# terraytherapeutics/COATI

Measured on AMD Instinct MI355X. Metric: molecules/sec (contrastive+AR train step), grande_closed, higher is better.
Workload: dtype bf16; 1 GPU; grande_closed d=256 L=16 nh=16 + E3GNN h=256x5, V=10322, batch 1024/GPU, seq_len 80, 16-atom point clouds, InfoNCE + AR loss, bf16 MFMA operands / fp32 accumulate + fp32 master weights, random-init weights; global_batch=1024, seq_len=80, parallelism=dp1

## Files before the change

### coati_amd/_lib.py

```python
import ctypes
import os

from . import _abi
from . import build as _build

try:
    with open(_build.HEADER) as _f:
        _ABI = _abi.parse(_f.read())
except OSError as e:
    raise RuntimeError(f"coati_amd: cannot read {_build.HEADER}, which the binding of libcoati_hip.so is derived from: {e}") from e
try:
    with open(_build.BEAM_HEADER) as _f:
        _BEAM_ABI = _abi.parse(_f.read(), guard="COATI_BEAM_H", name="coati_beam.h", base=_ABI)
except OSError as e:
    raise RuntimeError(f"coati_amd: cannot read {_build.BEAM_HEADER}, which the beam-search binding is derived from: {e}") from e
try:
    with open(_build.SEARCH_HEADER) as _f:
        _SEARCH_ABI = _abi.parse(_f.read(), guard="COATI_SEARCH_H", name="coati_search.h", base=_ABI)
except OSError as e:
    raise RuntimeError(f"coati_amd: cannot read {_build.SEARCH_HEADER}, which the library-search binding is derived from: {e}") from e
try:
    with open(_build.GRAMMAR_HEADER) as _f:
        _GRAMMAR_ABI = _abi.parse(_f.read(), guard="COATI_GRAMMAR_H", name="coati_grammar.h", base=_ABI)
except OSError as e:
# ... 61 lines not shown
try:
    with open(_build.PQ_HEADER) as _f:
        _PQ_ABI = _abi.parse(_f.read(), guard="COATI_PQ_H", name="coati_pq.h", base=_ABI)
except OSError as e:
    raise RuntimeError(f"coati_amd: cannot read {_build.PQ_HEADER}, which the binding of the product-quantised search is derived from: {e}") from e
try:
    with open(_build.IVFPQ_HEADER) as _f:
        _IVFPQ_ABI = _abi.parse(_f.read(), guard="COATI_IVFPQ_H", name="coati_ivfpq.h", base=_ABI)
except OSError as e:
    raise RuntimeError(f"coati_amd: cannot read {_build.IVFPQ_HEADER}, which the binding of the IVF-PQ search is derived from: {e}") from e
try:
    with open(_build.SEARCH4_HEADER) as _f:
        _SEARCH4_ABI = _abi.parse(_f.read(), guard="COATI_SEARCH4_H", name="coati_search4.h", base=_ABI)
except OSError as e:
    raise RuntimeError(f"coati_amd: cannot read {_build.SEARCH4_HEADER}, which the binding of the four-bit search is derived from: {e}") from e

PROTOTYPES = _ABI.prototypes
CoatiConfig = _ABI.CoatiConfig
ABI_VERSION = _ABI.version
BEAM_PROTOTYPES = _BEAM_ABI.prototypes
SEARCH_PROTOTYPES = _SEARCH_ABI.prototypes
GRAMMAR_PROTOTYPES = _GRAMMAR_ABI.prototypes
SCREEN_PROTOTYPES = _SCREEN_ABI.prototypes
GUIDE_PROTOTYPES = _GUIDE_ABI.prototypes
LN_XHAT_PROTOTYPES = _LN_XHAT_ABI.prototypes
GP_PROTOTYPES = _GP_ABI.prototypes
ACQ_PROTOTYPES = _ACQ_ABI.prototypes
CLUSTER_PROTOTYPES = _CLUSTER_ABI.prototypes
IVF_PROTOTYPES = _IVF_ABI.prototypes
RADIUS_PROTOTYPES = _RADIUS_ABI.prototypes
GNN_OPS_PROTOTYPES = _GNN_OPS_ABI.prototypes
SEARCH8_PROTOTYPES = _SEARCH8_ABI.prototypes
IVF8_PROTOTYPES = _IVF8_ABI.prototypes
IVF_RADIUS_PROTOTYPES = _IVF_RADIUS_ABI.prototypes
PQ_PROTOTYPES = _PQ_ABI.prototypes
IVFPQ_PROTOTYPES = _IVFPQ_ABI.prototypes
SEARCH4_PROTOTYPES = _SEARCH4_ABI.prototypes

_lib = None


def has_experimental():
    return hasattr(lib(), "coati_attn_block_fwd")


def lib():
    global _lib
    if _lib is not None:
        return _lib
    path = _build.LIB
    try:
        _build.build(force=os.environ.get("COATI_AMD_REBUILD") == "1", verbose=False)
    except Exception:
        if not os.path.exists(path):
            raise
    if not os.path.exists(path):
        raise RuntimeError(f"coati_amd: {path} is missing and could not be built; there is no CPU fallback")
    import torch
    l = ctypes.CDLL(path)
    for name, (restype, argtypes) in list(PROTOTYPES.items()) + list(BEAM_PROTOTYPES.items()) + list(SEARCH_PROTOTYPES.items()) + list(GRAMMAR_PROTOTYPES.items()) + list(SCREEN_PROTOTYPES.items()) + list(GUIDE_PROTOTYPES.items()) + list(LN_XHAT_PROTOTYPES.items()) + list(GP_PROTOTYPES.items()) + list(ACQ_PROTOTYPES.items()) + list(CLUSTER_PROTOTYPES.items()) + list(IVF_PROTOTYPES.items()) + list(RADIUS_PROTOTYPES.items()) + list(GNN_OPS_PROTOTYPES.items()) + list(SEARCH8_PROTOTYPES.items()) + list(IVF8_PROTOTYPES.items()) + list(IVF_RADIUS_PROTOTYPES.items()) + list(PQ_PROTOTYPES.items()) + list(IVFPQ_PROTOTYPES.items()) + list(SEARCH4_PROTOTYPES.items()):
        if hasattr(l, name):
            getattr(l, name).restype = restype
            getattr(l, name).argtypes = argtypes
    if l.coati_abi_version() != ABI_VERSION:
        raise RuntimeError(f"coati_amd: {path} has ABI version {l.coati_abi_version()}, this package expects {ABI_VERSION}; "
                           "rebuild with `python -m coati_amd.build --force`")
    missing = [n for n in exported_symbols() + sorted(BEAM_PROTOTYPES) + sorted(SEARCH_PROTOTYPES) + sorted(GRAMMAR_PROTOTYPES) + sorted(SCREEN_PROTOTYPES) + sorted(GUIDE_PROTOTYPES) + sorted(LN_XHAT_PROTOTYPES) + sorted(GP_PROTOTYPES) + sorted(ACQ_PROTOTYPES) + sorted(CLUSTER_PROTOTYPES) + sorted(IVF_PROTOTYPES) + sorted(RADIUS_PROTOTYPES) + sorted(GNN_OPS_PROTOTYPES) + sorted(SEARCH8_PROTOTYPES) + sorted(IVF8_PROTOTYPES) + sorted(IVF_RADIUS_PROTOTYPES) + sorted(PQ_PROTOTYPES) + sorted(IVFPQ_PROTOTYPES) + sorted(SEARCH4_PROTOTYPES) if not hasattr(l, n)]
    if missing:
        raise RuntimeError(f"coati_amd: {path} lacks symbols {missing[:6]}; rebuild with `python -m coati_amd.build --force`")
    _lib = l
    return l


def exported_symbols():
    return sorted(n for n in PROTOTYPES if _build.EXPERIMENTAL or n not in _ABI.experimental)


def check(rc, what=""):
    if rc != 0:
        msg = lib().coati_last_error().decode("utf-8", "replace")
        raise RuntimeError(f"libcoati_hip: {what} failed (code {rc}): {msg}")

# ... 6 lines not shown
```

### coati_amd/build.py

```python
import os
import subprocess
import sys
from concurrent.futures import ThreadPoolExecutor

HERE = os.path.dirname(os.path.abspath(__file__))
CSRC = os.path.join(HERE, "csrc")
LIBDIR = os.path.join(HERE, "lib")
LIB = os.path.join(LIBDIR, "libcoati_hip_x.so" if os.environ.get("COATI_AMD_EXPERIMENTAL") == "1" else "libcoati_hip.so")
OBJDIR = os.path.join(HERE, "build")
HEADER = os.path.join(os.path.dirname(HERE), "include", "coati_hip.h")
BEAM_HEADER = os.path.join(os.path.dirname(HERE), "include", "coati_beam.h")
SEARCH_HEADER = os.path.join(os.path.dirname(HERE), "include", "coati_search.h")
GRAMMAR_HEADER = os.path.join(os.path.dirname(HERE), "include", "coati_grammar.h")
SCREEN_HEADER = os.path.join(os.path.dirname(HERE), "include", "coati_screen.h")
GUIDE_HEADER = os.path.join(os.path.dirname(HERE), "include", "coati_guide.h")
LN_XHAT_HEADER = os.path.join(os.path.dirname(HERE), "include", "coati_ln_xhat.h")
GP_HEADER = os.path.join(os.path.dirname(HERE), "include", "coati_gp.h")
ACQ_HEADER = os.path.join(os.path.dirname(HERE), "include", "coati_acq.h")
CLUSTER_HEADER = os.path.join(os.path.dirname(HERE), "include", "coati_cluster.h")
IVF_HEADER = os.path.join(os.path.dirname(HERE), "include", "coati_ivf.h")
RADIUS_HEADER = os.path.join(os.path.dirname(HERE), "include", "coati_radius.h")
GNN_OPS_HEADER = os.path.join(os.path.dirname(HERE), "include", "coati_gnn_ops.h")
SEARCH8_HEADER = os.path.join(os.path.dirname(HERE), "include", "coati_search8.h")
IVF8_HEADER = os.path.join(os.path.dirname(HERE), "include", "coati_ivf8.h")
IVF_RADIUS_HEADER = os.path.join(os.path.dirname(HERE), "include", "coati_ivf_radius.h")
PQ_HEADER = os.path.join(os.path.dirname(HERE), "include", "coati_pq.h")
IVFPQ_HEADER = os.path.join(os.path.dirname(HERE), "include", "coati_ivfpq.h")
SEARCH4_HEADER = os.path.join(os.path.dirname(HERE), "include", "coati_search4.h")
HIP_UNITS = ["gemm.hip", "gemm_rb.hip", "gemm_rb16.hip", "gemm_ring.hip", "gemm_mx8.hip", "norm.hip", "attention.hip", "attention16.hip", "embed.hip", "gnn.hip", "loss.hip", "optim.hip", "batch.hip", "decode.hip", "beam.hip", "search.hip", "grammar.hip", "screen.hip", "guide.hip", "gp.hip", "gp_grad.hip", "cluster.hip", "ivf.hip", "radius.hip", "search8.hip", "ivf8.hip", "ivf_radius.hip", "pq.hip", "ivfpq.hip", "search4.hip"]
CPP_UNITS = ["engine.cpp", "capi.cpp", "tokenizer.cpp", "comm.cpp"]
FLAGS = ["--offload-arch=gfx950", "-O3", "-std=c++17", "-fPIC", "-Wno-unused-value", "-mllvm", "-amdgpu-mfma-vgpr-form=1"] + os.environ.get("COATI_AMD_CXXFLAGS", "").split()


EXPERIMENTAL = os.environ.get("COATI_AMD_EXPERIMENTAL") == "1"
EXPERIMENTAL_UNITS = ["experimental/attn_block.hip", "experimental/mlp64.hip", "experimental/gemm_t32.hip"]
if EXPERIMENTAL:
    HIP_UNITS = HIP_UNITS + EXPERIMENTAL_UNITS
    FLAGS = FLAGS + ["-DCOATI_EXPERIMENTAL"]
UNIT_DROP_FLAGS = {"experimental/mlp64.hip": ("-mllvm", "-amdgpu-mfma-vgpr-form=1")}


def _hipcc():
    for c in (os.environ.get("HIPCC"), "/opt/rocm/bin/hipcc", "hipcc"):
        if c and (os.path.isabs(c) and os.path.exists(c) or not os.path.isabs(c)):
            return c
    return "hipcc"


def _sources():
    deps = [os.path.join(CSRC, f) for f in os.listdir(CSRC) if not os.path.isdir(os.path.join(CSRC, f))]
    if EXPERIMENTAL:
        deps += [os.path.join(CSRC, "experimental", f) for f in os.listdir(os.path.join(CSRC, "experimental"))]
    deps += [HEADER, BEAM_HEADER, SEARCH_HEADER, GRAMMAR_HEADER, SCREEN_HEADER, GUIDE_HEADER, LN_XHAT_HEADER, GP_HEADER, ACQ_HEADER, CLUSTER_HEADER, IVF_HEADER, RADIUS_HEADER, GNN_OPS_HEADER, SEARCH8_HEADER, IVF8_HEADER, IVF_RADIUS_HEADER, PQ_HEADER, IVFPQ_HEADER, SEARCH4_HEADER]
    return deps


def _stamp_path():
    return LIB + ".flags"


def needs_build():
    if not os.path.exists(LIB):
        return True
    try:
        with open(_stamp_path()) as f:
            if f.read() != " ".join(FLAGS):
                return True
    except OSError:
# ... 51 lines not shown
```

### coati_amd/csrc/capi.cpp

```cpp
#include <string.h>

#include "../../include/coati_hip.h"
#include "../../include/coati_beam.h"
#include "../../include/coati_search.h"
#include "../../include/coati_grammar.h"
#include "../../include/coati_screen.h"
#include "../../include/coati_guide.h"
#include "../../include/coati_ln_xhat.h"
#include "../../include/coati_gp.h"
#include "../../include/coati_acq.h"
#include "../../include/coati_cluster.h"
#include "../../include/coati_ivf.h"
#include "../../include/coati_radius.h"
#include "../../include/coati_search8.h"
#include "../../include/coati_ivf8.h"
#include "../../include/coati_ivf_radius.h"
#include "../../include/coati_pq.h"
#include "../../include/coati_ivfpq.h"
#include "../../include/coati_search4.h"
#include "../../include/coati_gnn_ops.h"
#include <vector>
#include "kernels.h"

#define S_(x) ((hipStream_t)(x))
#define LL(x) (reinterpret_cast<const long long*>(x))

extern "C" {

int coati_gemm_nt(const void* A, int a_f32, int64_t lda, const uint16_t* B, int64_t ldb, int M, int N, int K,
                  void* C, int64_t ldc, int n_store, const float* bias, const void* aux_in, void* aux_out,
                  int64_t ld_aux, int epi, void* stream) {
  COATI_CHECK_ARG((epi >= EPI_BF16 && epi <= EPI_ACC_F32) || epi == EPI_GELU_GRAD || epi == EPI_MUL_AUX, "coati_gemm_nt: epilogue %d is not a plain epilogue", epi);
  GemmArgs a;
  memset(&a, 0, sizeof(a));
  a.A = A; a.lda = lda; a.B = B; a.ldb = ldb; a.M = M; a.N = N; a.K = K; a.C = C; a.ldc = ldc; a.n_store = n_store;
// ... 445 lines not shown
}
int coati_gnn_edge_reduce(const uint16_t* s2, const int32_t* seg, const float* e_w, uint16_t* mi, int64_t ldmi, int BA, int H, void* stream) {
  return launch_gnn_edge_reduce_c(s2, seg, e_w, mi, ldmi, BA, H, S_(stream));
}

int coati_gnn_edge_fwd_fused(const uint16_t* P, int64_t ldp, const int32_t* seg, const int32_t* e_bk, const float* e_d2, const float* e_w,
                             const float* w1c, int64_t w1c_stride, const float* b1, const uint16_t* W3, int64_t ldw, const float* b3,
                             uint16_t* e1, uint16_t* s2, uint16_t* mi, int64_t ldmi, int BA, int H, void* stream) {
  return launch_gnn_edge_fwd_fused(P, ldp, seg, e_bk, e_d2, e_w, w1c, w1c_stride, b1, W3, ldw, b3, e1, s2, mi, ldmi, BA, H, S_(stream));
}
int coati_gnn_edge_reduce_bwd(const uint16_t* dmi, int64_t lddmi, const uint16_t* s2, const int32_t* seg, const float* e_w, uint16_t* ds2,
                              int BA, int H, void* stream) {
  COATI_CHECK_SHAPE(BA > 0 && H > 0, "gnn_edge_reduce_bwd: empty problem");
  return launch_gnn_edge_reduce_bwd_c(dmi, lddmi, s2, seg, e_w, ds2, BA, H, S_(stream));
}
int coati_gnn_edge_pre_bwd(const uint16_t* dpre, const int32_t* seg, const int32_t* e_rev, const float* e_d2, uint16_t* dP, int64_t lddp,
                           float* dw1c, int64_t dw1c_stride, float* db1, int BA, int H, void* stream) {
  COATI_CHECK_SHAPE(BA > 0 && H > 0, "gnn_edge_pre_bwd: empty problem");
  return launch_gnn_edge_pre_bwd_c(dpre, seg, e_rev, e_d2, dP, lddp, dw1c, dw1c_stride, db1, BA, H, S_(stream));
}
int coati_gnn_node_res_silu(const float* u32, const int64_t* atoms, const int32_t* lut_ix, const int32_t* lut_iy, const float* W3c,
                            int64_t ldw, uint16_t* upre, uint16_t* t16, int BA, int H, void* stream) {
  COATI_CHECK_SHAPE(BA > 0 && H > 0, "gnn_node_res_silu: empty problem");
  return launch_gnn_node_res_silu(u32, LL(atoms), lut_ix, lut_iy, W3c, ldw, upre, t16, BA, H, S_(stream));
}
int coati_gnn_onehot_wgrad(const int64_t* atoms, const int32_t* lut_ix, const int32_t* lut_iy, const uint16_t* du, float* dW, int64_t ldw,
                           int BA, int H, void* stream) {
  COATI_CHECK_SHAPE(BA > 0 && H > 0, "gnn_onehot_wgrad: empty problem");
  return launch_gnn_onehot_wgrad(LL(atoms), lut_ix, lut_iy, du, dW, ldw, BA, H, S_(stream));
}
// ... 100 lines not shown
```

### coati_amd/csrc/engine.cpp

```cpp
#include <stdarg.h>
#include <stdio.h>
#include <stdlib.h>
#include <string.h>

#include <algorithm>
#include <string>
#include <vector>

#include "../../include/coati_hip.h"
#include "../../include/coati_beam.h"
#include "../../include/coati_ln_xhat.h"
#include "kernels.h"

#define HIPCHK(x) do { hipError_t _h = (x); if (_h != hipSuccess) { coati_set_error("%s: %s", #x, hipGetErrorString(_h)); return COATI_EHIP; } } while (0)

static thread_local char g_err[512] = "";
void coati_set_error(const char* fmt, ...) {
  va_list ap;
  va_start(ap, fmt);
  vsnprintf(g_err, sizeof(g_err), fmt, ap);
  va_end(ap);
}
extern "C" const char* coati_last_error(void) { return g_err; }
extern "C" int coati_abi_version(void) { return COATI_ABI_VERSION; }
// ... 1218 lines not shown
    bf16_t* const du = grp ? e->gl_du[l] : e->g_du;
    bf16_t* const dP = grp ? e->gl_dP[l] : e->g_dP;
    {
      ProfScope ps(e, SITE_GNN_ELEMWISE, 0, s, (double)BA * (H * 4 + H * 4 + 4 + H * 4 + H * 2));
      COATI_TRY(launch_layernorm_bwd(DH, 1, H, e->g_h32[l + 1], H, 1, nullptr, e->g_rstd[l + 1], nullptr, nullptr, DO, DO16, nullptr, nullptr, e->ln_partial, BA, H, s));
    }
    COATI_TRY(gemm(e, SITE_GNN_NODE_GEMM, DO16, 0, H, e->S + w.n3T, H, BA, H, H, du, H, nullptr, EPI_DSILU, e->g_upre[l], nullptr, H, s));
    if (!grp) COATI_TRY(wgrad(e, SITE_GNN_WGRAD, DO16, 0, H, e->g_t[l], H, BA, H, H, e->G + w.n3w, H, e->G + w.n3b, 0, s));
    COATI_TRY(gemm(e, SITE_GNN_NODE_GEMM, du, 0, H, e->S + w.n0T, H, BA, H, H, DO, H, nullptr, EPI_ACC_F32, nullptr, nullptr, 0, s));
    COATI_TRY(gemm(e, SITE_GNN_NODE_GEMM, du, 0, H, e->S + w.n0T + (int64_t)H * H, H, BA, H, H, e->g_dmi, H, nullptr, EPI_BF16, nullptr, nullptr, 0, s));
    if (!grp) COATI_TRY(wgrad(e, SITE_GNN_WGRAD, du, 0, H, e->g_hcat[l], 2 * H, BA, H, 2 * H, e->G + w.n0w, 2 * H + (c.residual ? 28 : 0), e->G + w.n0b, 0, s));
    if (c.residual) {
      ProfScope ps(e, SITE_GNN_ELEMWISE, 0, s, (double)BA * (H * 2 + 8));
      COATI_TRY(launch_gnn_onehot_wgrad(e->atoms, e->lut_ix, e->lut_iy, du, e->G + w.n0w + 2 * H, 2 * H + 28, BA, H, s));
    }
    {
      ProfScope ps(e, SITE_GNN_ELEMWISE, 0, s, (double)BA * (H * 2 + 4), (double)H * 4 + 4, 6.0 * H);
      COATI_TRY(launch_gnn_edge_reduce_bwd_c(e->g_dmi, H, e->g_s2[l], e->g_seg, e->g_ew, e->g_ds2, BA, H, s));
    }
    {
      GemmArgs a;
      memset(&a, 0, sizeof(a));
      a.A = e->g_ds2; a.lda = H; a.B = e->S + w.e3T; a.ldb = H; a.M = Me; a.N = H; a.K = H; a.C = e->g_dpre1; a.ldc = H;
      a.P = e->g_P[l]; a.ldp = 2 * H; a.d2 = e->g_ed2; a.w1c = e->P + w.e0w + 2 * H; a.w1c_stride = 2 * H + 1;
      a.b1 = e->P + w.e0b; a.natom = A; a.H = H;
      a.m_dev = e->g_ne; a.e_bj = e->g_ebj; a.e_bk = e->g_ebk;
      ProfScope ps(e, SITE_GNN_EDGE_GEMM, 0, s, (double)H * H * 2, (double)H * 8 + 12, 2.0 * H * H + 8.0 * H);
      COATI_TRY(launch_gemm_nt(a, 0, EPI_EDGE_DPRE, s));
    }
    {
      WgradArgs a;
      a.A = e->g_ds2; a.lda = H; a.B = e->g_e1[l]; a.ldb = H; a.M = Me; a.N = H; a.K = H; a.dW = e->G + w.e3w; a.ldw = H; a.dbias = e->G + w.e3b;
      a.n_out = 0; a.m_dev = e->g_ne;
      ProfScope ps(e, SITE_GNN_WGRAD, 0, s, (double)H * H * 8, (double)H * 4, 2.0 * H * H);
      COATI_TRY(launch_wgrad(a, 0, s));
    }
    {
      ProfScope ps(e, SITE_GNN_ELEMWISE, 0, s, (double)BA * (H * 4 + 4), (double)H * 4 + 8, 4.0 * H);
      COATI_TRY(launch_gnn_edge_pre_bwd_c(e->g_dpre1, e->g_seg, e->g_erev, e->g_ed2, dP, 2 * H, e->G + w.e0w + 2 * H, 2 * H + 1, e->G + w.e0b, BA, H, s));
    }
    COATI_TRY(gemm(e, SITE_GNN_NODE_GEMM, dP, 0, 2 * H, e->S + w.w1abT, 2 * H, BA, H, 2 * H, DO, H, nullptr, EPI_ACC_F32, nullptr, nullptr, 0, s));
    if (!grp) {
      COATI_TRY(wgrad(e, SITE_GNN_WGRAD, dP, 0, 2 * H, e->g_hcat[l], 2 * H, BA, H, H, e->G + w.e0w, 2 * H + 1, nullptr, 0, s));
// ... 1192 lines not shown
```

### coati_amd/csrc/gemm_rb16.hip

```cpp
#include <algorithm>
#include <cstdlib>
#include "gemm_epi.h"

#define R16_K 256
#define R16_BN 64
#define R16_TILE_HALFS (R16_BN * R16_K)
#define R16_BIAS_MAX 4096
#define R16_MAXW 16
#ifndef R16_TURNS
#define R16_TURNS 4
#endif
#ifndef R16_PRIO
#define R16_PRIO 0
#endif
#ifndef R16_ABLATE
#define R16_ABLATE 0
#endif
typedef float f32x4_t __attribute__((ext_vector_type(4)));
typedef unsigned r16_v4u __attribute__((ext_vector_type(4)));
#if R16_ABLATE & 16
__device__ unsigned char r16_sink[512 * 4096];
#endif

template <typename F>
// ... 335 lines not shown
    sm += __shfl_xor(sm, 16, 64);
    sm += __shfl_xor(sm, 32, 64);
    if (rowok && kq == 0) p.lse_out[row_l] = mx + __logf(sm);
    if (p.tl_out != nullptr) {
      float tl = ce_tl + __shfl_xor(ce_tl, 16, 64);
      tl += __shfl_xor(tl, 32, 64);
      if (rowok && kq == 0) p.tl_out[row_l] = tl;
    }
  }
#if R16_ABLATE & 16
#undef p
#endif
}

#define R16_RES_TILES 4
template <int EPI>
__global__ __launch_bounds__(64 * R16_MAXW, 1) void gemm_rb16_resident_kernel(GemmArgs p) {
  extern __shared__ __attribute__((aligned(16))) unsigned char smem[];
  constexpr int MAP = 0;
  bf16_t* const Bs = reinterpret_cast<bf16_t*>(smem);
  float* const BiasS = reinterpret_cast<float*>(smem + R16_RES_TILES * R16_TILE_HALFS * 2);
  float* const ColS = BiasS + R16_RES_TILES * R16_BN;
  const int tid = threadIdx.x, lane = tid & 63, wave = __builtin_amdgcn_readfirstlane(tid >> 6), W = blockDim.x >> 6;
  const int fr = lane & 15, kq = lane >> 4;
  const int ntiles = (p.N + R16_BN - 1) / R16_BN;
  const int M = __builtin_amdgcn_readfirstlane(p.m_dev != nullptr ? *p.m_dev : p.M);
  const bool has_bias = p.bias != nullptr;
  if (M <= 0) return;
  for (int c = tid; c < ntiles * R16_BN; c += blockDim.x) {
    BiasS[c] = (has_bias && c < p.N) ? p.bias[c] : 0.f;
// ... 10 lines not shown
    const int gc = r < p.N ? r : p.N - 1;
    const bf16_t* src = p.B + (long long)gc * p.ldb + ((q ^ r16_swz<MAP>(r & 63)) * 8);
    __builtin_amdgcn_global_load_lds((gbl_void*)src, (lds_void*)(Bs + k * 512), 16, 0, 0);
  }
  __builtin_amdgcn_s_waitcnt(0x0f70);
  __syncthreads();

  int wofs[4], wsw[4];
#pragma unroll
  for (int a = 0; a < 4; ++a) {
    const int n = r16_wrow<MAP>(a, fr);
    wofs[a] = n * R16_K;
    wsw[a] = r16_swz<MAP>(n);
  }
  const int colA = 8 * kq, colB = 32 + 8 * kq;
  GemmArgs q = p;
  q.bias = nullptr;
  q.M = M;

  const int slabs = (M + 15) / 16, per_wg = (slabs + (int)gridDim.x - 1) / (int)gridDim.x;
  const int s_begin = blockIdx.x * per_wg, s_end = s_begin + per_wg < slabs ? s_begin + per_wg : slabs;
  for (int sl = s_begin + wave; sl < s_end; sl += W) {
    const int m0 = sl * 16, row_l = m0 + fr, rc = row_l < M ? row_l : M - 1;
    const bool rowok = row_l < M;
    bf16x8 af[8];
    {
      const bf16_t* ap = reinterpret_cast<const bf16_t*>(p.A) + (long long)rc * p.lda + kq * 8;
#pragma unroll
      for (int ks = 0; ks < 8; ++ks) af[ks] = *reinterpret_cast<const bf16x8*>(ap + ks * 32);
    }
    for (int jt = 0; jt < ntiles; ++jt) {
      const bf16_t* cur = Bs + jt * R16_TILE_HALFS;
      f32x4_t acc[4];
      acc[0] = *reinterpret_cast<const f32x4_t*>(BiasS + jt * R16_BN + colA);
      acc[1] = *reinterpret_cast<const f32x4_t*>(BiasS + jt * R16_BN + colA + 4);
      acc[2] = *reinterpret_cast<const f32x4_t*>(BiasS + jt * R16_BN + colB);
      acc[3] = *reinterpret_cast<const f32x4_t*>(BiasS + jt * R16_BN + colB + 4);
      {
        constexpr int WFD = (EPI == EPI_EDGE_DPRE) ? 1 : 2;
// ... 6 lines not shown
#pragma unroll
            for (int a = 0; a < 4; ++a) wf[(ks + 1) % WFD][a] = *reinterpret_cast<const bf16x8*>(cur + wofs[a] + (((4 * (ks + 1) + kq) ^ wsw[a]) * 8));
          }
#pragma unroll
          for (int a = 0; a < 4; ++a) acc[a] = __builtin_amdgcn_mfma_f32_16x16x32_bf16(wf[ks % WFD][a], af[ks], acc[a], 0, 0, 0);
          if (WFD == 1 && ks + 1 < 8) {
#pragma unroll
            for (int a = 0; a < 4; ++a) wf[0][a] = *reinterpret_cast<const bf16x8*>(cur + wofs[a] + (((4 * (ks + 1) + kq) ^ wsw[a]) * 8));
          }
          __builtin_amdgcn_sched_barrier(0);
        }
      }
      float v0[8] = {acc[0][0], acc[0][1], acc[0][2], acc[0][3], acc[1][0], acc[1][1], acc[1][2], acc[1][3]};
      float v1[8] = {acc[2][0], acc[2][1], acc[2][2], acc[2][3], acc[3][0], acc[3][1], acc[3][2], acc[3][3]};
      const int c0 = jt * R16_BN + colA, c1 = jt * R16_BN + colB;
      const void* st0 = nullptr;
      const void* st1 = nullptr;
      if constexpr (EPI == EPI_EDGE_DPRE) { st0 = ColS + jt * 128 + colA; st1 = ColS + jt * 128 + colB; }
      epilogue8<EPI>(q, row_l, c0, v0, rowok, jt, ntiles, st0);
      __builtin_amdgcn_sched_barrier(0);
      epilogue8<EPI>(q, row_l, c1, v1, rowok, jt, ntiles, st1);
    }
  }
}

bool gemm_rb16_resident_supported(const GemmArgs& a, int a_f32, int epi) {
  if (a_f32 || a.K != R16_K || a.m_dev == nullptr) return false;
  if (epi != EPI_BF16 && epi != EPI_EDGE_DPRE) return false;
  if (a.N % 16 != 0 || a.N > R16_RES_TILES * R16_BN || a.q8_out != nullptr || a.ln_x != nullptr) return false;
  return a.M >= 16 * 256;
}

template <int EPI>
static int launch_rb16_resident_t(const GemmArgs& a, hipStream_t s) {
  static bool attr_set = false;
  auto kern = gemm_rb16_resident_kernel<EPI>;
  constexpr size_t lds = (size_t)R16_RES_TILES * R16_TILE_HALFS * 2 + (size_t)R16_RES_TILES * R16_BN * 4 + (size_t)R16_RES_TILES * 128 * 4;
  if (!attr_set) {
    if (hipFuncSetAttribute(reinterpret_cast<const void*>(kern), hipFuncAttributeMaxDynamicSharedMemorySize, (int)lds) != hipSuccess) {
      coati_set_error("gemm_rb16(resident): hipFuncSetAttribute failed");
      return COATI_EHIP;
    }
    attr_set = true;
  }
  hipLaunchKernelGGL(kern, dim3(256), dim3(64 * R16_MAXW), lds, s, a);
  COATI_LAUNCH_CHECK("gemm_rb16_resident");
  return COATI_OK;
}

int launch_gemm_rb16_resident(const GemmArgs& a, int epi, hipStream_t s) {
  if (epi == EPI_EDGE_DPRE) return launch_rb16_resident_t<EPI_EDGE_DPRE>(a, s);
  return launch_rb16_resident_t<EPI_BF16>(a, s);
}

template <int CTRL>
__device__ __forceinline__ float r16_dpp(float v) {
  return __builtin_bit_cast(float, __builtin_amdgcn_update_dpp(0, __builtin_bit_cast(int, v), CTRL, 0xf, 0xf, false));
}
__device__ __forceinline__ float r16_row_sum(float v) {
  v += r16_dpp<0xB1>(v);
  v += r16_dpp<0x4E>(v);
  v += r16_dpp<0x141>(v);
  v += r16_dpp<0x140>(v);
  return v;
}

struct GnnEdgeFwdArgs {
// ... 220 lines not shown
```

### coati_amd/csrc/kernels.h

```cpp
#pragma once
#include "common.h"

enum CoatiEpi {
  EPI_BF16 = 0,
  EPI_F32 = 1,
  EPI_RES_F32 = 2,
  EPI_GELU = 3,
  EPI_DGELU = 4,
  EPI_SILU = 5,
  EPI_DSILU = 6,
  EPI_ACC_F32 = 7,
  EPI_CE_PARTIAL = 8,
  EPI_CE_BWD = 9,
  EPI_EDGE_DPRE = 10,
  EPI_QKV_ROPE = 11,
  EPI_GELU_GRAD = 12,
  EPI_MUL_AUX = 13,
  EPI_LNBWD = 14,
  EPI_CE_BWD_ROW = 15,
  EPI_CE_LSE = 16,
  EPI_COUNT = 17
};

struct GemmArgs {
// ... 344 lines not shown
                             bf16_t* upre, bf16_t* t16, int BA, int H, hipStream_t s);
int launch_gnn_onehot_wgrad(const long long* atoms, const int* lut_ix, const int* lut_iy, const bf16_t* du, float* dW, long long ldw, int BA,
                            int H, hipStream_t s);
int launch_gnn_embed_bwd(const long long* atoms, const int* lut_ix, const int* lut_iy, const float* de,
                         float* dW, float* db, int BA, int H, hipStream_t s);
int launch_gnn_geom(const float* coords, const float* mask, float cutoff, float* d2, float* w, int B, int A,
                    hipStream_t s);
int launch_gnn_compact(const float* w_dense, const float* d2_dense, int* seg, int* n_edges, int* e_bj, int* e_bk, int* e_rev,
                       float* e_d2, float* e_w, int* pos, int B, int A, hipStream_t s);
int launch_gnn_edge_pre_c(const bf16_t* P, long long ldp, const int* seg, const int* e_bk, const float* e_d2, const float* w1c,
                          long long w1c_stride, const float* b1, bf16_t* e1, int BA, int H, hipStream_t s);
int launch_gnn_edge_reduce_c(const bf16_t* s2, const int* seg, const float* e_w, bf16_t* mi, long long ldmi, int BA, int H, hipStream_t s);
int launch_gnn_edge_fwd_fused(const bf16_t* P, long long ldp, const int* seg, const int* e_bk, const float* e_d2, const float* e_w,
                              const float* w1c, long long w1c_stride, const float* b1, const bf16_t* W3, long long ldw, const float* b3,
                              bf16_t* e1, bf16_t* s2, bf16_t* mi, long long ldmi, int BA, int H, hipStream_t s);
int launch_gnn_edge_reduce_bwd_c(const bf16_t* dmi, long long lddmi, const bf16_t* s2, const int* seg, const float* e_w,
                                 bf16_t* ds2, int BA, int H, hipStream_t s);
int launch_gnn_edge_pre_bwd_c(const bf16_t* dpre, const int* seg, const int* e_rev, const float* e_d2, bf16_t* dP, long long lddp,
                              float* dw1c, long long dw1c_stride, float* db1, int BA, int H, hipStream_t s);
int launch_gnn_readout(const float* o, const float* mask, float* hp, int B, int A, int H, hipStream_t s);
int launch_gnn_readout_bwd(const float* dhp, const float* mask, bf16_t* dout, int B, int A, int H, hipStream_t s);

int launch_silu_fwd(const float* x, float* y, long long n, hipStream_t s);
int launch_silu_bwd(const float* x, const float* dy, float* dx, long long n, int accumulate, hipStream_t s);
int launch_swiglu(const float* u, long long ldu, float* g, long long ldg, int B, int N, hipStream_t s);
int launch_swiglu_bwd(const float* u, long long ldu, const float* dg, long long lddg, float* du, long long lddu, int B, int N, hipStream_t s);
int launch_group_mean_rows(const float* x, long long ldx, const int* off, const float* w, const float* fallback, float* out, int G, int E,
                           hipStream_t s);
int launch_select_rows(const unsigned char* use_a, const float* a, const float* b, float* out, int B, int C,
                       hipStream_t s);
// ... 33 lines not shown
```

Measured before the change: 50360 molecules/s.

## Fuse GNN edge reduce-backward into the resident edge dpre GEMM kernel

```diff
diff --git a/coati_amd/_lib.py b/coati_amd/_lib.py
--- a/coati_amd/_lib.py
+++ b/coati_amd/_lib.py
@@ -99,6 +99,11 @@
         _SEARCH4_ABI = _abi.parse(_f.read(), guard="COATI_SEARCH4_H", name="coati_search4.h", base=_ABI)
 except OSError as e:
     raise RuntimeError(f"coati_amd: cannot read {_build.SEARCH4_HEADER}, which the binding of the four-bit search is derived from: {e}") from e
+try:
+    with open(_build.GNN_EDGE_BWD_HEADER) as _f:
+        _GNN_EDGE_BWD_ABI = _abi.parse(_f.read(), guard="COATI_GNN_EDGE_BWD_H", name="coati_gnn_edge_bwd.h", base=_ABI)
+except OSError as e:
+    raise RuntimeError(f"coati_amd: cannot read {_build.GNN_EDGE_BWD_HEADER}, which the binding of the fused backward edge launch is derived from: {e}") from e
 
 PROTOTYPES = _ABI.prototypes
 CoatiConfig = _ABI.CoatiConfig
@@ -121,6 +126,7 @@
 PQ_PROTOTYPES = _PQ_ABI.prototypes
 IVFPQ_PROTOTYPES = _IVFPQ_ABI.prototypes
 SEARCH4_PROTOTYPES = _SEARCH4_ABI.prototypes
+GNN_EDGE_BWD_PROTOTYPES = _GNN_EDGE_BWD_ABI.prototypes
 
 _lib = None
 
@@ -143,14 +149,14 @@
         raise RuntimeError(f"coati_amd: {path} is missing and could not be built; there is no CPU fallback")
     import torch
     l = ctypes.CDLL(path)
-    for name, (restype, argtypes) in list(PROTOTYPES.items()) + list(BEAM_PROTOTYPES.items()) + list(SEARCH_PROTOTYPES.items()) + list(GRAMMAR_PROTOTYPES.items()) + list(SCREEN_PROTOTYPES.items()) + list(GUIDE_PROTOTYPES.items()) + list(LN_XHAT_PROTOTYPES.items()) + list(GP_PROTOTYPES.items()) + list(ACQ_PROTOTYPES.items()) + list(CLUSTER_PROTOTYPES.items()) + list(IVF_PROTOTYPES.items()) + list(RADIUS_PROTOTYPES.items()) + list(GNN_OPS_PROTOTYPES.items()) + list(SEARCH8_PROTOTYPES.items()) + list(IVF8_PROTOTYPES.items()) + list(IVF_RADIUS_PROTOTYPES.items()) + list(PQ_PROTOTYPES.items()) + list(IVFPQ_PROTOTYPES.items()) + list(SEARCH4_PROTOTYPES.items()):
+    for name, (restype, argtypes) in list(PROTOTYPES.items()) + list(BEAM_PROTOTYPES.items()) + list(SEARCH_PROTOTYPES.items()) + list(GRAMMAR_PROTOTYPES.items()) + list(SCREEN_PROTOTYPES.items()) + list(GUIDE_PROTOTYPES.items()) + list(LN_XHAT_PROTOTYPES.items()) + list(GP_PROTOTYPES.items()) + list(ACQ_PROTOTYPES.items()) + list(CLUSTER_PROTOTYPES.items()) + list(IVF_PROTOTYPES.items()) + list(RADIUS_PROTOTYPES.items()) + list(GNN_OPS_PROTOTYPES.items()) + list(SEARCH8_PROTOTYPES.items()) + list(IVF8_PROTOTYPES.items()) + list(IVF_RADIUS_PROTOTYPES.items()) + list(PQ_PROTOTYPES.items()) + list(IVFPQ_PROTOTYPES.items()) + list(SEARCH4_PROTOTYPES.items()) + list(GNN_EDGE_BWD_PROTOTYPES.items()):
         if hasattr(l, name):
             getattr(l, name).restype = restype
             getattr(l, name).argtypes = argtypes
     if l.coati_abi_version() != ABI_VERSION:
         raise RuntimeError(f"coati_amd: {path} has ABI version {l.coati_abi_version()}, this package expects {ABI_VERSION}; "
                            "rebuild with `python -m coati_amd.build --force`")
-    missing = [n for n in exported_symbols() + sorted(BEAM_PROTOTYPES) + sorted(SEARCH_PROTOTYPES) + sorted(GRAMMAR_PROTOTYPES) + sorted(SCREEN_PROTOTYPES) + sorted(GUIDE_PROTOTYPES) + sorted(LN_XHAT_PROTOTYPES) + sorted(GP_PROTOTYPES) + sorted(ACQ_PROTOTYPES) + sorted(CLUSTER_PROTOTYPES) + sorted(IVF_PROTOTYPES) + sorted(RADIUS_PROTOTYPES) + sorted(GNN_OPS_PROTOTYPES) + sorted(SEARCH8_PROTOTYPES) + sorted(IVF8_PROTOTYPES) + sorted(IVF_RADIUS_PROTOTYPES) + sorted(PQ_PROTOTYPES) + sorted(IVFPQ_PROTOTYPES) + sorted(SEARCH4_PROTOTYPES) if not hasattr(l, n)]
+    missing = [n for n in exported_symbols() + sorted(BEAM_PROTOTYPES) + sorted(SEARCH_PROTOTYPES) + sorted(GRAMMAR_PROTOTYPES) + sorted(SCREEN_PROTOTYPES) + sorted(GUIDE_PROTOTYPES) + sorted(LN_XHAT_PROTOTYPES) + sorted(GP_PROTOTYPES) + sorted(ACQ_PROTOTYPES) + sorted(CLUSTER_PROTOTYPES) + sorted(IVF_PROTOTYPES) + sorted(RADIUS_PROTOTYPES) + sorted(GNN_OPS_PROTOTYPES) + sorted(SEARCH8_PROTOTYPES) + sorted(IVF8_PROTOTYPES) + sorted(IVF_RADIUS_PROTOTYPES) + sorted(PQ_PROTOTYPES) + sorted(IVFPQ_PROTOTYPES) + sorted(SEARCH4_PROTOTYPES) + sorted(GNN_EDGE_BWD_PROTOTYPES) if not hasattr(l, n)]
     if missing:
         raise RuntimeError(f"coati_amd: {path} lacks symbols {missing[:6]}; rebuild with `python -m coati_amd.build --force`")
     _lib = l
diff --git a/coati_amd/build.py b/coati_amd/build.py
--- a/coati_amd/build.py
+++ b/coati_amd/build.py
@@ -27,6 +27,7 @@
 PQ_HEADER = os.path.join(os.path.dirname(HERE), "include", "coati_pq.h")
 IVFPQ_HEADER = os.path.join(os.path.dirname(HERE), "include", "coati_ivfpq.h")
 SEARCH4_HEADER = os.path.join(os.path.dirname(HERE), "include", "coati_search4.h")
+GNN_EDGE_BWD_HEADER = os.path.join(os.path.dirname(HERE), "include", "coati_gnn_edge_bwd.h")
 HIP_UNITS = ["gemm.hip", "gemm_rb.hip", "gemm_rb16.hip", "gemm_ring.hip", "gemm_mx8.hip", "norm.hip", "attention.hip", "attention16.hip", "embed.hip", "gnn.hip", "loss.hip", "optim.hip", "batch.hip", "decode.hip", "beam.hip", "search.hip", "grammar.hip", "screen.hip", "guide.hip", "gp.hip", "gp_grad.hip", "cluster.hip", "ivf.hip", "radius.hip", "search8.hip", "ivf8.hip", "ivf_radius.hip", "pq.hip", "ivfpq.hip", "search4.hip"]
 CPP_UNITS = ["engine.cpp", "capi.cpp", "tokenizer.cpp", "comm.cpp"]
 FLAGS = ["--offload-arch=gfx950", "-O3", "-std=c++17", "-fPIC", "-Wno-unused-value", "-mllvm", "-amdgpu-mfma-vgpr-form=1"] + os.environ.get("COATI_AMD_CXXFLAGS", "").split()
@@ -51,7 +52,7 @@
     deps = [os.path.join(CSRC, f) for f in os.listdir(CSRC) if not os.path.isdir(os.path.join(CSRC, f))]
     if EXPERIMENTAL:
         deps += [os.path.join(CSRC, "experimental", f) for f in os.listdir(os.path.join(CSRC, "experimental"))]
-    deps += [HEADER, BEAM_HEADER, SEARCH_HEADER, GRAMMAR_HEADER, SCREEN_HEADER, GUIDE_HEADER, LN_XHAT_HEADER, GP_HEADER, ACQ_HEADER, CLUSTER_HEADER, IVF_HEADER, RADIUS_HEADER, GNN_OPS_HEADER, SEARCH8_HEADER, IVF8_HEADER, IVF_RADIUS_HEADER, PQ_HEADER, IVFPQ_HEADER, SEARCH4_HEADER]
+    deps += [HEADER, BEAM_HEADER, SEARCH_HEADER, GRAMMAR_HEADER, SCREEN_HEADER, GUIDE_HEADER, LN_XHAT_HEADER, GP_HEADER, ACQ_HEADER, CLUSTER_HEADER, IVF_HEADER, RADIUS_HEADER, GNN_OPS_HEADER, SEARCH8_HEADER, IVF8_HEADER, IVF_RADIUS_HEADER, PQ_HEADER, IVFPQ_HEADER, SEARCH4_HEADER, GNN_EDGE_BWD_HEADER]
     return deps
 
 
diff --git a/coati_amd/csrc/capi.cpp b/coati_amd/csrc/capi.cpp
--- a/coati_amd/csrc/capi.cpp
+++ b/coati_amd/csrc/capi.cpp
@@ -19,6 +19,7 @@
 #include "../../include/coati_ivfpq.h"
 #include "../../include/coati_search4.h"
 #include "../../include/coati_gnn_ops.h"
+#include "../../include/coati_gnn_edge_bwd.h"
 #include <vector>
 #include "kernels.h"
 
@@ -494,6 +495,13 @@
   COATI_CHECK_SHAPE(BA > 0 && H > 0, "gnn_edge_reduce_bwd: empty problem");
   return launch_gnn_edge_reduce_bwd_c(dmi, lddmi, s2, seg, e_w, ds2, BA, H, S_(stream));
 }
+int coati_gnn_edge_bwd_fused(const int32_t* m_dev, const uint16_t* s2, const uint16_t* dmi, int64_t lddmi, const int32_t* e_bj,
+                             const int32_t* e_bk, const float* e_d2, const float* e_w, const uint16_t* W, int64_t ldw, const uint16_t* P,
+                             int64_t ldp, const float* w1c, int64_t w1c_stride, const float* b1, uint16_t* ds2, uint16_t* dpre, int cap, int BA,
+                             int H, int grid, void* stream) {
+  return launch_gnn_edge_bwd_fused(m_dev, s2, dmi, lddmi, e_bj, e_bk, e_d2, e_w, W, ldw, P, ldp, w1c, w1c_stride, b1, ds2, dpre, cap, BA, H, grid,
+                                   S_(stream));
+}
 int coati_gnn_edge_pre_bwd(const uint16_t* dpre, const int32_t* seg, const int32_t* e_rev, const float* e_d2, uint16_t* dP, int64_t lddp,
                            float* dw1c, int64_t dw1c_stride, float* db1, int BA, int H, void* stream) {
   COATI_CHECK_SHAPE(BA > 0 && H > 0, "gnn_edge_pre_bwd: empty problem");
diff --git a/coati_amd/csrc/engine.cpp b/coati_amd/csrc/engine.cpp
--- a/coati_amd/csrc/engine.cpp
+++ b/coati_amd/csrc/engine.cpp
@@ -1256,19 +1256,23 @@
       ProfScope ps(e, SITE_GNN_ELEMWISE, 0, s, (double)BA * (H * 2 + 8));
       COATI_TRY(launch_gnn_onehot_wgrad(e->atoms, e->lut_ix, e->lut_iy, du, e->G + w.n0w + 2 * H, 2 * H + 28, BA, H, s));
     }
-    {
-      ProfScope ps(e, SITE_GNN_ELEMWISE, 0, s, (double)BA * (H * 2 + 4), (double)H * 4 + 4, 6.0 * H);
-      COATI_TRY(launch_gnn_edge_reduce_bwd_c(e->g_dmi, H, e->g_s2[l], e->g_seg, e->g_ew, e->g_ds2, BA, H, s));
-    }
-    {
-      GemmArgs a;
-      memset(&a, 0, sizeof(a));
-      a.A = e->g_ds2; a.lda = H; a.B = e->S + w.e3T; a.ldb = H; a.M = Me; a.N = H; a.K = H; a.C = e->g_dpre1; a.ldc = H;
-      a.P = e->g_P[l]; a.ldp = 2 * H; a.d2 = e->g_ed2; a.w1c = e->P + w.e0w + 2 * H; a.w1c_stride = 2 * H + 1;
-      a.b1 = e->P + w.e0b; a.natom = A; a.H = H;
-      a.m_dev = e->g_ne; a.e_bj = e->g_ebj; a.e_bk = e->g_ebk;
+    GemmArgs ea;
+    memset(&ea, 0, sizeof(ea));
+    ea.A = e->g_ds2; ea.lda = H; ea.B = e->S + w.e3T; ea.ldb = H; ea.M = Me; ea.N = H; ea.K = H; ea.C = e->g_dpre1; ea.ldc = H;
+    ea.P = e->g_P[l]; ea.ldp = 2 * H; ea.d2 = e->g_ed2; ea.w1c = e->P + w.e0w + 2 * H; ea.w1c_stride = 2 * H + 1;
+    ea.b1 = e->P + w.e0b; ea.natom = A; ea.H = H;
+    ea.m_dev = e->g_ne; ea.e_bj = e->g_ebj; ea.e_bk = e->g_ebk;
+    if (H == 256 && gemm_rb16_resident_supported(ea, 0, EPI_EDGE_DPRE)) {
+      ProfScope ps(e, SITE_GNN_EDGE_GEMM, 0, s, (double)H * H * 2 + (double)BA * H * 2, (double)H * 10 + 16, 2.0 * H * H + 14.0 * H);
+      COATI_TRY(launch_gnn_edge_bwd_fused(e->g_ne, e->g_s2[l], e->g_dmi, H, e->g_ebj, e->g_ebk, e->g_ed2, e->g_ew, e->S + w.e3T, H, e->g_P[l], 2 * H,
+                                          e->P + w.e0w + 2 * H, 2 * H + 1, e->P + w.e0b, e->g_ds2, e->g_dpre1, Me, BA, H, 0, s));
+    } else {
+      {
+        ProfScope ps(e, SITE_GNN_ELEMWISE, 0, s, (double)BA * (H * 2 + 4), (double)H * 4 + 4, 6.0 * H);
+        COATI_TRY(launch_gnn_edge_reduce_bwd_c(e->g_dmi, H, e->g_s2[l], e->g_seg, e->g_ew, e->g_ds2, BA, H, s));
+      }
       ProfScope ps(e, SITE_GNN_EDGE_GEMM, 0, s, (double)H * H * 2, (double)H * 8 + 12, 2.0 * H * H + 8.0 * H);
-      COATI_TRY(launch_gemm_nt(a, 0, EPI_EDGE_DPRE, s));
+      COATI_TRY(launch_gemm_nt(ea, 0, EPI_EDGE_DPRE, s));
     }
     {
       WgradArgs a;
diff --git a/coati_amd/csrc/gemm_rb16.hip b/coati_amd/csrc/gemm_rb16.hip
--- a/coati_amd/csrc/gemm_rb16.hip
+++ b/coati_amd/csrc/gemm_rb16.hip
@@ -373,6 +373,24 @@
 }
 
 #define R16_RES_TILES 4
+
+__device__ __forceinline__ void r16_edge_dpre8(const bf16_t* __restrict__ P, unsigned offa, unsigned offb, float d2, const float* wc,
+                                               const float* bc, const float (&v)[8], bf16_t* __restrict__ C, unsigned coff, bool rowok) {
+  const uint4 ua = *reinterpret_cast<const uint4*>(P + offa), ub = *reinterpret_cast<const uint4*>(P + offb);
+  float pa[8], pb[8], o[8];
+  unpack8(ua, pa);
+  unpack8(ub, pb);
+  const float4 w0 = *reinterpret_cast<const float4*>(wc), w1 = *reinterpret_cast<const float4*>(wc + 4);
+  const float4 b0 = *reinterpret_cast<const float4*>(bc), b1 = *reinterpret_cast<const float4*>(bc + 4);
+  const float wv[8] = {w0.x, w0.y, w0.z, w0.w, w1.x, w1.y, w1.z, w1.w}, bv[8] = {b0.x, b0.y, b0.z, b0.w, b1.x, b1.y, b1.z, b1.w};
+#pragma unroll
+  for (int e = 0; e < 8; ++e) {
+    const float pre = pa[e] + pb[e] + d2 * wv[e] + bv[e];
+    o[e] = v[e] * dsilu_f(pre);
+  }
+  if (rowok) *reinterpret_cast<uint4*>(C + coff) = pack8(o);
+}
+
 template <int EPI>
 __global__ __launch_bounds__(64 * R16_MAXW, 1) void gemm_rb16_resident_kernel(GemmArgs p) {
   extern __shared__ __attribute__((aligned(16))) unsigned char smem[];
@@ -413,15 +431,27 @@
     wsw[a] = r16_swz<MAP>(n);
   }
   const int colA = 8 * kq, colB = 32 + 8 * kq;
-  GemmArgs q = p;
-  q.bias = nullptr;
-  q.M = M;
 
   const int slabs = (M + 15) / 16, per_wg = (slabs + (int)gridDim.x - 1) / (int)gridDim.x;
   const int s_begin = blockIdx.x * per_wg, s_end = s_begin + per_wg < slabs ? s_begin + per_wg : slabs;
   for (int sl = s_begin + wave; sl < s_end; sl += W) {
     const int m0 = sl * 16, row_l = m0 + fr, rc = row_l < M ? row_l : M - 1;
     const bool rowok = row_l < M;
+    unsigned offa = 0, offb = 0;
+    float d2 = 0.f;
+    if constexpr (EPI == EPI_EDGE_DPRE) {
+      int bj, bk;
+      if (p.e_bj) {
+        bj = p.e_bj[rc];
+        bk = p.e_bk[rc];
+      } else {
+        bj = rc / p.natom;
+        bk = (rc / (p.natom * p.natom)) * p.natom + (rc - bj * p.natom);
+      }
+      offa = (unsigned)bj * (unsigned)p.ldp;
+      offb = (unsigned)bk * (unsigned)p.ldp + (unsigned)p.H;
+      d2 = p.d2[rc];
+    }
     bf16x8 af[8];
     {
       const bf16_t* ap = reinterpret_cast<const bf16_t*>(p.A) + (long long)rc * p.lda + kq * 8;
@@ -458,12 +488,19 @@
       float v0[8] = {acc[0][0], acc[0][1], acc[0][2], acc[0][3], acc[1][0], acc[1][1], acc[1][2], acc[1][3]};
       float v1[8] = {acc[2][0], acc[2][1], acc[2][2], acc[2][3], acc[3][0], acc[3][1], acc[3][2], acc[3][3]};
       const int c0 = jt * R16_BN + colA, c1 = jt * R16_BN + colB;
-      const void* st0 = nullptr;
-      const void* st1 = nullptr;
-      if constexpr (EPI == EPI_EDGE_DPRE) { st0 = ColS + jt * 128 + colA; st1 = ColS + jt * 128 + colB; }
-      epilogue8<EPI>(q, row_l, c0, v0, rowok, jt, ntiles, st0);
-      __builtin_amdgcn_sched_barrier(0);
-      epilogue8<EPI>(q, row_l, c1, v1, rowok, jt, ntiles, st1);
+      if constexpr (EPI == EPI_EDGE_DPRE) {
+        bf16_t* C = reinterpret_cast<bf16_t*>(p.C);
+        const unsigned coff = (unsigned)rc * (unsigned)p.ldc;
+        r16_edge_dpre8(p.P, offa + c0, offb + c0, d2, ColS + jt * 128 + colA, ColS + jt * 128 + 64 + colA, v0, C, coff + c0, rowok);
+        __builtin_amdgcn_sched_barrier(0);
+        r16_edge_dpre8(p.P, offa + c1, offb + c1, d2, ColS + jt * 128 + colB, ColS + jt * 128 + 64 + colB, v1, C, coff + c1, rowok);
+      } else {
+        GemmArgs q = p;
+        q.bias = nullptr;
+        q.M = M;
+        epilogue8<EPI>(q, row_l, c0, v0, rowok, jt, ntiles);
+        epilogue8<EPI>(q, row_l, c1, v1, rowok, jt, ntiles);
+      }
     }
   }
 }
@@ -472,6 +509,7 @@
   if (a_f32 || a.K != R16_K || a.m_dev == nullptr) return false;
   if (epi != EPI_BF16 && epi != EPI_EDGE_DPRE) return false;
   if (a.N % 16 != 0 || a.N > R16_RES_TILES * R16_BN || a.q8_out != nullptr || a.ln_x != nullptr) return false;
+  if (epi == EPI_EDGE_DPRE && (a.N != R16_K || a.H != a.N || a.n_store > a.N || (long long)a.M * a.ldp >= (1ll << 31) || (long long)a.M * a.ldc >= (1ll << 31))) return false;
   return a.M >= 16 * 256;
 }
 
@@ -495,6 +533,142 @@
 int launch_gemm_rb16_resident(const GemmArgs& a, int epi, hipStream_t s) {
   if (epi == EPI_EDGE_DPRE) return launch_rb16_resident_t<EPI_EDGE_DPRE>(a, s);
   return launch_rb16_resident_t<EPI_BF16>(a, s);
+}
+
+struct GnnEdgeBwdArgs {
+  const int* m_dev;
+  const bf16_t* s2;
+  const bf16_t* dmi; unsigned lddmi;
+  const int* e_bj; const int* e_bk; const float* e_d2; const float* e_w;
+  const bf16_t* W; unsigned ldw;
+  const bf16_t* P; unsigned ldp;
+  const float* w1c; long long w1c_stride; const float* b1;
+  bf16_t* ds2; bf16_t* dpre;
+};
+
+#ifndef R16_EDGE_DS2_NT
+#define R16_EDGE_DS2_NT 0
+#endif
+__global__ __launch_bounds__(64 * R16_MAXW, 1) void gnn_edge_bwd_fused_kernel(GnnEdgeBwdArgs p) {
+  extern __shared__ __attribute__((aligned(16))) unsigned char smem[];
+  constexpr int MAP = 0, H = R16_K, NT = R16_RES_TILES;
+  bf16_t* const Bs = reinterpret_cast<bf16_t*>(smem);
+  float* const K1 = reinterpret_cast<float*>(smem + NT * R16_TILE_HALFS * 2);
+  const int tid = threadIdx.x, lane = tid & 63, wave = __builtin_amdgcn_readfirstlane(tid >> 6), W = blockDim.x >> 6;
+  const int fr = lane & 15, kq = lane >> 4;
+  const int M = __builtin_amdgcn_readfirstlane(*p.m_dev);
+  if (M <= 0) return;
+  for (int c = tid; c < H; c += blockDim.x) {
+    K1[c] = p.w1c[(long long)c * p.w1c_stride];
+    K1[H + c] = p.b1[c];
+  }
+  typedef __attribute__((address_space(3))) void lds_void;
+  typedef __attribute__((address_space(1))) const void gbl_void;
+  for (int k = wave; k < NT * (R16_BN / 2); k += W) {
+    const int r = 2 * k + (lane >> 5), q = lane & 31;
+    const bf16_t* src = p.W + (unsigned)r * p.ldw + ((q ^ r16_swz<MAP>(r & 63)) * 8);
+    __builtin_amdgcn_global_load_lds((gbl_void*)src, (lds_void*)(Bs + k * 512), 16, 0, 0);
+  }
+  __builtin_amdgcn_s_waitcnt(0x0f70);
+  __syncthreads();
+
+  int wb[4];
+#pragma unroll
+  for (int a = 0; a < 4; ++a) {
+    const int n = r16_wrow<MAP>(a, fr);
+    wb[a] = n * R16_K + ((kq ^ r16_swz<MAP>(n)) * 8);
+  }
+  const int colA = 8 * kq, colB = 32 + 8 * kq;
+
+  const int slabs = (M + 15) / 16, per_wg = (slabs + (int)gridDim.x - 1) / (int)gridDim.x;
+  const int s_begin = blockIdx.x * per_wg, s_end = s_begin + per_wg < slabs ? s_begin + per_wg : slabs;
+  for (int sl = s_begin + wave; sl < s_end; sl += W) {
+    const int row_l = sl * 16 + fr;
+    const bool rowok = row_l < M;
+    const unsigned rc = rowok ? row_l : M - 1;
+    const unsigned bj = p.e_bj[rc], bk = p.e_bk[rc];
+    const float d2 = p.e_d2[rc], w = p.e_w[rc];
+    bf16x8 af[8];
+    {
+      const bf16_t* sp = p.s2 + (rc * (unsigned)H + kq * 8);
+      const bf16_t* gp = p.dmi + (bj * p.lddmi + kq * 8);
+      bf16_t* dp = p.ds2 + (rc * (unsigned)H + kq * 8);
+#pragma unroll
+      for (int ks = 0; ks < 8; ++ks) {
+        const uint4 us = *reinterpret_cast<const uint4*>(sp + ks * 32), ug = *reinterpret_cast<const uint4*>(gp + ks * 32);
+        float x[8], g[8], o[8];
+        unpack8(us, x);
+        unpack8(ug, g);
+#pragma unroll
+        for (int i = 0; i < 8; ++i) o[i] = g[i] * w * dsilu_f(x[i]);
+        uint4 u = pack8(o);
+        if (rowok) {
+#if R16_EDGE_DS2_NT
+          __builtin_nontemporal_store(r16_v4u{u.x, u.y, u.z, u.w}, reinterpret_cast<r16_v4u*>(dp + ks * 32));
+#else
+          *reinterpret_cast<uint4*>(dp + ks * 32) = u;
+#endif
+        } else {
+          u = make_uint4(0u, 0u, 0u, 0u);
+        }
+        af[ks] = __builtin_bit_cast(bf16x8, u);
+      }
+    }
+    const unsigned offa = bj * p.ldp, offb = bk * p.ldp + H, coff = rc * (unsigned)H;
+    for (int jt = 0; jt < NT; ++jt) {
+      const bf16_t* cur = Bs + jt * R16_TILE_HALFS;
+      f32x4_t acc[4];
+#pragma unroll
+      for (int a = 0; a < 4; ++a) acc[a] = f32x4_t{0.f, 0.f, 0.f, 0.f};
+      {
+        bf16x8 wf[4];
+#pragma unroll
+        for (int a = 0; a < 4; ++a) wf[a] = *reinterpret_cast<const bf16x8*>(cur + wb[a]);
+#pragma unroll
+        for (int ks = 0; ks < 8; ++ks) {
+#pragma unroll
+          for (int a = 0; a < 4; ++a) acc[a] = __builtin_amdgcn_mfma_f32_16x16x32_bf16(wf[a], af[ks], acc[a], 0, 0, 0);
+          if (ks + 1 < 8) {
+#pragma unroll
+            for (int a = 0; a < 4; ++a) wf[a] = *reinterpret_cast<const bf16x8*>(cur + (wb[a] ^ ((ks + 1) * 32)));
+          }
+          __builtin_amdgcn_sched_barrier(0);
+        }
+      }
+      const float v0[8] = {acc[0][0], acc[0][1], acc[0][2], acc[0][3], acc[1][0], acc[1][1], acc[1][2], acc[1][3]};
+      const float v1[8] = {acc[2][0], acc[2][1], acc[2][2], acc[2][3], acc[3][0], acc[3][1], acc[3][2], acc[3][3]};
+      const int c0 = jt * R16_BN + colA, c1 = jt * R16_BN + colB;
+      r16_edge_dpre8(p.P, offa + c0, offb + c0, d2, K1 + c0, K1 + H + c0, v0, p.dpre, coff + c0, rowok);
+      __builtin_amdgcn_sched_barrier(0);
+      r16_edge_dpre8(p.P, offa + c1, offb + c1, d2, K1 + c1, K1 + H + c1, v1, p.dpre, coff + c1, rowok);
+    }
+  }
+}
+
+int launch_gnn_edge_bwd_fused(const int* m_dev, const bf16_t* s2, const bf16_t* dmi, long long lddmi, const int* e_bj, const int* e_bk,
+                              const float* e_d2, const float* e_w, const bf16_t* W, long long ldw, const bf16_t* P, long long ldp,
+                              const float* w1c, long long w1c_stride, const float* b1, bf16_t* ds2, bf16_t* dpre, int cap, int BA, int H,
+                              int grid, hipStream_t s) {
+  COATI_CHECK_ARG(m_dev && s2 && dmi && e_bj && e_bk && e_d2 && e_w && W && P && w1c && b1 && ds2 && dpre, "gnn_edge_bwd_fused: null operand");
+  COATI_CHECK_SHAPE(H == R16_K && BA > 0 && cap > 0 && grid >= 0 && lddmi >= H && lddmi % 8 == 0 && ldw >= H && ldw % 8 == 0 && ldp >= 2 * H && ldp % 8 == 0,
+                    "gnn_edge_bwd_fused: H = 256 only (H=%d)", H);
+  COATI_CHECK_SHAPE((long long)cap * H < (1ll << 31) && (long long)BA * ldp < (1ll << 31) && (long long)BA * lddmi < (1ll << 31) && ldw * H < (1ll << 31),
+                    "gnn_edge_bwd_fused: operand too large for 32-bit offsets (cap=%d BA=%d)", cap, BA);
+  static bool attr_set = false;
+  constexpr size_t lds = (size_t)R16_RES_TILES * R16_TILE_HALFS * 2 + (size_t)R16_K * 4 * 2;
+  if (!attr_set) {
+    if (hipFuncSetAttribute(reinterpret_cast<const void*>(gnn_edge_bwd_fused_kernel), hipFuncAttributeMaxDynamicSharedMemorySize, (int)lds) != hipSuccess) {
+      coati_set_error("gnn_edge_bwd_fused: hipFuncSetAttribute failed");
+      return COATI_EHIP;
+    }
+    attr_set = true;
+  }
+  GnnEdgeBwdArgs a;
+  a.m_dev = m_dev; a.s2 = s2; a.dmi = dmi; a.lddmi = (unsigned)lddmi; a.e_bj = e_bj; a.e_bk = e_bk; a.e_d2 = e_d2; a.e_w = e_w;
+  a.W = W; a.ldw = (unsigned)ldw; a.P = P; a.ldp = (unsigned)ldp; a.w1c = w1c; a.w1c_stride = w1c_stride; a.b1 = b1; a.ds2 = ds2; a.dpre = dpre;
+  hipLaunchKernelGGL(gnn_edge_bwd_fused_kernel, dim3(grid > 0 ? grid : 256), dim3(64 * R16_MAXW), lds, s, a);
+  COATI_LAUNCH_CHECK("gnn_edge_bwd_fused");
+  return COATI_OK;
 }
 
 template <int CTRL>
diff --git a/coati_amd/csrc/kernels.h b/coati_amd/csrc/kernels.h
--- a/coati_amd/csrc/kernels.h
+++ b/coati_amd/csrc/kernels.h
@@ -382,6 +382,10 @@
 int launch_gnn_edge_fwd_fused(const bf16_t* P, long long ldp, const int* seg, const int* e_bk, const float* e_d2, const float* e_w,
                               const float* w1c, long long w1c_stride, const float* b1, const bf16_t* W3, long long ldw, const float* b3,
                               bf16_t* e1, bf16_t* s2, bf16_t* mi, long long ldmi, int BA, int H, hipStream_t s);
+int launch_gnn_edge_bwd_fused(const int* m_dev, const bf16_t* s2, const bf16_t* dmi, long long lddmi, const int* e_bj, const int* e_bk,
+                              const float* e_d2, const float* e_w, const bf16_t* W, long long ldw, const bf16_t* P, long long ldp,
+                              const float* w1c, long long w1c_stride, const float* b1, bf16_t* ds2, bf16_t* dpre, int cap, int BA, int H,
+                              int grid, hipStream_t s);
 int launch_gnn_edge_reduce_bwd_c(const bf16_t* dmi, long long lddmi, const bf16_t* s2, const int* seg, const float* e_w,
                                  bf16_t* ds2, int BA, int H, hipStream_t s);
 int launch_gnn_edge_pre_bwd_c(const bf16_t* dpre, const int* seg, const int* e_rev, const float* e_d2, bf16_t* dP, long long lddp,
diff --git a/include/coati_gnn_edge_bwd.h b/include/coati_gnn_edge_bwd.h
--- /dev/null
+++ b/include/coati_gnn_edge_bwd.h
@@ -0,0 +1,19 @@
+#ifndef COATI_GNN_EDGE_BWD_H
+#define COATI_GNN_EDGE_BWD_H
+
+#include "coati_hip.h"
+
+#ifdef __cplusplus
+extern "C" {
+#endif
+
+int coati_gnn_edge_bwd_fused(const int32_t* m_dev, const uint16_t* s2, const uint16_t* dmi, int64_t lddmi, const int32_t* e_bj,
+                             const int32_t* e_bk, const float* e_d2, const float* e_w, const uint16_t* W, int64_t ldw, const uint16_t* P,
+                             int64_t ldp, const float* w1c, int64_t w1c_stride, const float* b1, uint16_t* ds2, uint16_t* dpre, int cap, int BA,
+                             int H, int grid, void* stream);
+
+#ifdef __cplusplus
+}
+#endif
+
+#endif
```

New measurement: 50520 molecules/s (median of 6 runs). About the same (+0.3%).
